# wei-zeng98/piano-a2s

Measured on AMD Instinct MI355X. Metric: training clips/sec (12 s, 5-bar), higher is better.
Workload: dtype f32

## Files before the change

piano_a2s_amd/csrc/a2s_api.hip:

```cpp
#define A2S_SWITCHES_IMPL
#include "a2s_internal.h"

thread_local char a2s_err_msg[512] = {0};
long long a2s_launch_counter = 0;

#define ST ((hipStream_t)stream)

extern "C" {

const char* a2s_last_error(void) { return a2s_err_msg; }
int a2s_version(void) { return 1; }
long long a2s_launch_count(void) { return __atomic_load_n(&a2s_launch_counter, __ATOMIC_RELAXED); }

int a2s_gemm_f32(void* stream, int M, int N, int K, float alpha, const float* A, long sAm, long sAk, const float* B, long sBk,
                 long sBn, float beta, float* C, long ldc, const float* bias, int act, int batch, long bsA, long bsB, long bsC,
                 int splitk, float* workspace, size_t workspace_bytes) {
    return a2s_gemm_impl(ST, M, N, K, alpha, A, sAm, sAk, B, sBk, sBn, beta, C, ldc, bias, act, batch, bsA, bsB, bsC, splitk,
                         workspace, workspace_bytes);
}
int a2s_gemm_f32_affine(void* stream, int M, int N, int K, float alpha, const float* A, long sAm, long sAk, const float* B, long sBk,
                        long sBn, float beta, float* C, long ldc, const float* bias, int act, int batch, long bsA, long bsB, long bsC,
                        int splitk, float* workspace, size_t workspace_bytes, const float* a_scale, const float* a_shift, int a_period,
                        const float* b_scale, const float* b_shift, int b_period) {
    return a2s_gemm_affine_impl(ST, M, N, K, alpha, A, sAm, sAk, B, sBk, sBn, beta, C, ldc, bias, act, batch, bsA, bsB, bsC, splitk,
// ... 30 lines not shown
                     const float* shift, int period, const float* dz_absmax, const float* y_absmax, float* workspace, size_t workspace_bytes) {
    return a2s_linear_wgrad_impl(ST, M, N, K, dz, ldz, y, lda, G, ldg, scale, shift, period, dz_absmax, y_absmax, workspace, workspace_bytes);
}
size_t a2s_linear_wgrad_ws_bytes(int M, int K) { return a2s_linear_wgrad_ws_bytes_impl(M, K); }
int a2s_linear_wgrad_eligible(int M, int N, int K, int period) { return a2s_linear_wgrad_ok(M, N, K, 256, 4, 4, period, nullptr, nullptr, nullptr) ? 1 : 0; }
int a2s_tallk_wgrad(void* stream, int M, int Np, int K, const float* P, long ldp, const float* A, long lda, float* G, long ldg, int transposed, float* bias,
                    const float* p_absmax, const float* a_absmax, float* workspace, size_t workspace_bytes) {
    return a2s_tallk_wgrad_impl(ST, M, Np, K, P, ldp, A, lda, G, ldg, transposed, bias, p_absmax, a_absmax, workspace, workspace_bytes);
}
size_t a2s_tallk_wgrad_ws_bytes(int M, int Np, int K) { return a2s_tallk_wgrad_ws_bytes_impl(M, Np, K); }
int a2s_tallk_wgrad_eligible(int M, int Np, int K, long ldp, long lda, long ldg, int transposed) {
    return a2s_tallk_wgrad_ok(M, Np, K, ldp, lda, ldg, transposed, nullptr, nullptr, nullptr, nullptr) ? 1 : 0;
}
int a2s_linear_fwd_eligible(int M, int N, int K, int period) { return a2s_linear_fwd_ok(M, N, K, 4, 4, period, nullptr, nullptr, nullptr) ? 1 : 0; }
int a2s_linear_dgrad_blocks(int M) { return a2s_linear_dgrad_blocks_impl(M); }
int a2s_linear_dgrad_eligible(int M, int N, int K, int period) {
    return a2s_linear_dgrad_ok(M, N, K, 4, 1, K, 4, period, nullptr, nullptr, nullptr, nullptr) ? 1 : 0;
}
int a2s_gemm_f32_bnstats(void* stream, int M, int N, int K, const float* A, long sAm, long sAk, const float* B, long sBk, long sBn, float* C, long ldc,
                         const float* y, const float* mean, const float* invstd, const float* scale, const float* shift, int period, float* partial) {
    return a2s_gemm_affine_impl(ST, M, N, K, 1.f, A, sAm, sAk, B, sBk, sBn, 0.f, C, ldc, nullptr, 0, 1, 0, 0, 0, 1, nullptr, 0,
                                nullptr, nullptr, 0, nullptr, nullptr, 0, y, mean, invstd, scale, shift, partial, period, 0, nullptr, nullptr);
}
int a2s_gemm_bnstats_blocks(int M, int period) { return a2s_cdiv(M, 128) * a2s_gemm_bnstats_slots(period); }
size_t a2s_gemm_workspace_bytes(int M, int N, int batch, int splitk) { return a2s_gemm_workspace_bytes_impl(M, N, batch, splitk); }
int a2s_gemm_pick_splitk(int M, int N, int K, int batch) { return a2s_gemm_pick_splitk_impl(M, N, K, batch); }
void a2s_gemm_debug_tile(int cfg) { a2s_gemm_debug_tile_impl(cfg); }
size_t a2s_note_step_workspace_floats(int H, int E) { return a2s_note_step_workspace_floats_impl(H, E); }
int a2s_debug_set(const char* key, int value) {
    if (!key) return A2S_ERR_ARG;
    const int id = a2s_switch_find(key);
    if (id >= 0) { a2s_switch_store(id, value); return A2S_OK; }
    if (!strcmp(key, "attn_deferred_fast")) { a2s_attn_deferred_fast = value ? 1 : 0; return A2S_OK; }
    if (!strcmp(key, "tallk_wgrad")) { a2s_tallk_wgrad_on = value ? 1 : 0; return A2S_OK; }
    if (!strcmp(key, "tallk_wgrad_max_splits")) { a2s_tallk_wgrad_max_splits = value > 0 ? value : 0; return A2S_OK; }
    if (!strcmp(key, "gemm_tile")) { a2s_gemm_debug_tile_impl(value); return A2S_OK; }
    snprintf(a2s_err_msg, sizeof(a2s_err_msg), "a2s_debug_set: unknown key %s", key);
    return A2S_ERR_ARG;
}
int a2s_env_check(void) {
    if (const char* e = a2s_switch_env_error()) A2S_FAIL(A2S_ERR_ARG, "%s: expected a decimal number >= 0", e);
    return A2S_OK;
}

int a2s_persist_abort_latch(void* device_word) { a2s_persist_latch_set(device_word); return A2S_OK; }

int a2s_debug_get(const char* key) {
    if (!key) return -1;
    const int id = a2s_switch_find(key);
    if (id == A2S_SW_attn_pair_fused_rows) return a2s_attn_pair_fused_rows();
    if (id >= 0) return a2s_sw((a2s_switch)id);
    if (!strcmp(key, "attn_pair_launches")) return (int)a2s_attn_pair_launches();
    if (!strcmp(key, "attn_pair_bwd_launches")) return (int)a2s_attn_pair_bwd_launches();
    if (!strcmp(key, "attn_deferred_fast")) return a2s_attn_deferred_fast;
    if (!strcmp(key, "tallk_wgrad")) return a2s_tallk_wgrad_on;
    if (!strcmp(key, "tallk_wgrad_max_splits")) return a2s_tallk_wgrad_max_splits;
    if (!strcmp(key, "tallk_wgrad_launches")) return (int)a2s_tallk_wgrad_launches();
    if (!strcmp(key, "attn_dk_ahead_launches")) return (int)a2s_attn_dk_ahead_launches();
    if (!strcmp(key, "attn_denc_launches")) return (int)a2s_attn_denc_launches();
    if (!strcmp(key, "dec_mid_launches")) return a2s_dec_mid_launches();
    if (!strcmp(key, "dec_cmb_launches")) return a2s_dec_cmb_launches();
    if (!strcmp(key, "dec_persist_launches")) return a2s_dec_persist_launches();
    if (!strcmp(key, "edit_distance_launches")) return (int)a2s_edit_distance_launches();
    if (!strcmp(key, "conv_rows16_c20_launches")) return (int)a2s_conv_rows16_c20_launches();
    if (!strcmp(key, "device_cus")) return a2s_device_geometry().cus;
    if (!strcmp(key, "device_xccs")) return a2s_device_geometry().xccs;
    return -1;
}

int a2s_conv3x3(void* stream, const float* x, const float* w, float* y, const float* in_scale, const float* in_shift,
                float* stat_partial, int B, int T, int F, int Cin, int Cout, int flip, float* workspace) {
    return a2s_conv3x3_impl(ST, x, w, y, in_scale, in_shift, stat_partial, B, T, F, Cin, Cout, flip, workspace, nullptr, nullptr, nullptr, nullptr, nullptr, nullptr,
                            nullptr, nullptr);
}
int a2s_conv3x3_ranged(void* stream, const float* x, const float* w, float* y, const float* in_scale, const float* in_shift, const float* in_absmax,
                       float* stat_partial, float* out_absmax, int B, int T, int F, int Cin, int Cout, float* workspace) {
    return a2s_conv3x3_impl(ST, x, w, y, in_scale, in_shift, stat_partial, B, T, F, Cin, Cout, 0, workspace, nullptr, nullptr, nullptr, nullptr, nullptr, nullptr,
                            in_absmax, out_absmax);
}
int a2s_conv3x3_dgrad_bnstats(void* stream, const float* dy, const float* w, float* g, const float* yl, const float* yl_mean, const float* yl_invstd,
                              const float* yl_scale, const float* yl_shift, float* stat_partial, int B, int T, int F, int Cin, int Cout,
                              float* workspace) {
    if (!yl) { snprintf(a2s_err_msg, sizeof(a2s_err_msg), "conv3x3_dgrad_bnstats: yl is required"); return A2S_ERR_ARG; }
    return a2s_conv3x3_impl(ST, dy, w, g, nullptr, nullptr, stat_partial, B, T, F, Cin, Cout, 1, workspace, yl, yl_mean, yl_invstd, yl_scale, yl_shift, nullptr, nullptr, nullptr);
}
int a2s_conv3x3_dgrad_bnstats_scaled(void* stream, const float* dy, const float* w, float* g, const float* yl, const float* yl_mean, const float* yl_invstd,
                                     const float* yl_scale, const float* yl_shift, float* stat_partial, int B, int T, int F, int Cin, int Cout,
                                     float* workspace, const float* dy_absmax) {
    if (!yl) { snprintf(a2s_err_msg, sizeof(a2s_err_msg), "conv3x3_dgrad_bnstats_scaled: yl is required"); return A2S_ERR_ARG; }
    return a2s_conv3x3_impl(ST, dy, w, g, nullptr, nullptr, stat_partial, B, T, F, Cin, Cout, 1, workspace, yl, yl_mean, yl_invstd, yl_scale, yl_shift, dy_absmax, nullptr, nullptr);
}
int a2s_conv3x3_dgrad_bnstats_ranged(void* stream, const float* dy, const float* w, float* g, const float* yl, const float* yl_mean, const float* yl_invstd,
                                     const float* yl_scale, const float* yl_shift, float* stat_partial, int B, int T, int F, int Cin, int Cout,
                                     float* workspace, const float* dy_absmax, float* g_absmax_out) {
    if (!yl) { snprintf(a2s_err_msg, sizeof(a2s_err_msg), "conv3x3_dgrad_bnstats_ranged: yl is required"); return A2S_ERR_ARG; }
    return a2s_conv3x3_impl(ST, dy, w, g, nullptr, nullptr, stat_partial, B, T, F, Cin, Cout, 1, workspace, yl, yl_mean, yl_invstd, yl_scale, yl_shift, dy_absmax, nullptr, g_absmax_out);
}
int a2s_bn_bwd_from_partial(void* stream, const float* g, const float* x, const float* mean, const float* invstd, const float* scale, const float* shift,
                            float* dgamma, float* dbeta, float* dx, const float* partial, int nblocks, float* c12, long rows, int C, int F) {
    return a2s_bn_bwd_from_partial_impl(ST, g, x, mean, invstd, scale, shift, dgamma, dbeta, dx, partial, nblocks, c12, rows, C, F, nullptr);
}
int a2s_bn_bwd_from_partial_amax(void* stream, const float* g, const float* x, const float* mean, const float* invstd, const float* scale, const float* shift,
                                 float* dgamma, float* dbeta, float* dx, const float* partial, int nblocks, float* c12, long rows, int C, int F,
                                 float* dx_absmax) {
    return a2s_bn_bwd_from_partial_impl(ST, g, x, mean, invstd, scale, shift, dgamma, dbeta, dx, partial, nblocks, c12, rows, C, F, dx_absmax);
}
// ... 360 lines not shown
```

piano_a2s_amd/csrc/a2s_bwd.hip:

```cpp
#include "a2s_internal.h"

__global__ __launch_bounds__(256) void log_softmax_bwd_rows(const float* __restrict__ g, const float* __restrict__ y,
                                                            long outer_stride, int inner, float* __restrict__ dx,
                                                            int R, int V, int n_outer, int time_major) {
    const int row = blockIdx.x * 4 + (threadIdx.x >> 6), lane = threadIdx.x & 63;
    if (row >= R) return;
    const int ob = row / inner, in = row % inner;
    const float* gr = g + (long)ob * outer_stride + (long)in * V;
    const float* yr = y + (long)ob * outer_stride + (long)in * V;
    float s = 0.f;
    for (int j = lane; j < V; j += 64) s += gr[j];
    s = wave_sum(s);
    const long orow = time_major ? ((long)in * n_outer + ob) : row;
    for (int j = lane; j < V; j += 64) dx[orow * V + j] = gr[j] - expf(yr[j]) * s;
}

int a2s_log_softmax_bwd_rows_impl(hipStream_t st, const float* g, const float* y, long outer_stride, int inner, float* dx,
                                  int R, int V, int n_outer, int time_major) {
    hipLaunchKernelGGL(log_softmax_bwd_rows, dim3(a2s_cdiv(R, 4)), dim3(256), 0, st, g, y, outer_stride, inner, dx, R, V, n_outer, time_major);
    A2S_CHECK_LAUNCH("log_softmax_bwd_rows");
    return A2S_OK;
}

__global__ void gru_gates_bwd(const float* __restrict__ dh_a, long lda, const float* __restrict__ dh_b, long ldb,
// ... 1086 lines not shown
    auto tile = [&](const f32x4 (&k)[4]) {
#pragma unroll
        for (int j = 0; j < NQ; ++j) {
            if (!on[j]) continue;
#pragma unroll
            for (int u = 0; u < 4; ++u) {
                const float w = dsv[j * chunk + i + 4 * u];
#pragma unroll
                for (int c = 0; c < 4; ++c) acc[j][c] = fmaf(w, sech2_ek(k[u][c], q4[j][c]), acc[j][c]);
            }
        }
    };
#pragma unroll
    for (int p = 0; p < KPRE; ++p)
        if (i + 12 < n) { tile(kpre[p]); i += 16; }
    for (; i + 12 < n; i += 16) {
        f32x4 k[4];
#pragma unroll
        for (int u = 0; u < 4; ++u) k[u] = ld_kv<NT>(Kb + (long)(i + 4 * u) * H + c4 * 4);
        tile(k);
    }
    for (; i < n; i += 4) {
        const f32x4 k0 = ld_kv<NT>(Kb + (long)i * H + c4 * 4);
#pragma unroll
        for (int j = 0; j < NQ; ++j) {
            if (!on[j]) continue;
            const float w = dsv[j * chunk + i];
#pragma unroll
            for (int c = 0; c < 4; ++c) acc[j][c] = fmaf(w, sech2_ek(k0[c], q4[j][c]), acc[j][c]);
        }
    }
    if (rg > 0) {
#pragma unroll
        for (int j = 0; j < NQ; ++j) red4[(j * 3 + rg - 1) * 64 + c4] = acc[j];
    }
    __syncthreads();
    if (rg == 0) {
        const f32x4 v4 = {v[c4 * 4], v[c4 * 4 + 1], v[c4 * 4 + 2], v[c4 * 4 + 3]};
#pragma unroll
        for (int j = 0; j < NQ; ++j) {
            if (!on[j]) continue;
            f32x4 a = acc[j];
#pragma unroll
            for (int u = 0; u < 3; ++u) { const f32x4 o = red4[(j * 3 + u) * 64 + c4];
#pragma unroll
                for (int c = 0; c < 4; ++c) a[c] += o[c]; }
#pragma unroll
            for (int c = 0; c < 4; ++c) a[c] *= v4[c];
            *reinterpret_cast<f32x4*>(dq_partial + (((long)slot * NQ + j) * G + g) * H + c4 * 4) = a;
        }
    }
}

struct AttnPairBwdSide { const float* Kmat; const float* q; const float* v; const float* attw; const float* ctx; const float* dctx_a; const float* dctx_b;
                         float* dctx_out; float* dq_partial; float* ds_out; const int* row_until; };
template <int NQ, bool NT>
__global__ __launch_bounds__(256, ATT_BWD_MQ_WAVES) void attn_bwd_split256_pair(AttnPairBwdSide s0, AttnPairBwdSide s1, const float* __restrict__ enc, long ldq,
                                                                                 long ldctx, long ldda, long lddb, long lddo, int T, int G, int chunk,
                                                                                 const int* __restrict__ clip_order, int step, int n_clips) {
    constexpr int H = 256, NJ = 2 * NQ;
    extern __shared__ __attribute__((aligned(16))) float sm[];
    float* dsv = sm;
    f32x4* red4 = reinterpret_cast<f32x4*>(sm + NJ * chunk);
    const int slot = blockIdx.x / G, g = blockIdx.x % G;
    const int b = clip_order ? clip_order[slot] : slot;
    const int t0 = g * chunk, t1 = min(T, t0 + chunk), n = t1 - t0;
    const int tid = threadIdx.x, lane = tid & 63, wave = tid >> 6;
    int onmask = 0;
#pragma unroll
    for (int j = 0; j < NQ; ++j) {
        onmask |= (!s0.row_until || step < s0.row_until[j * n_clips + b]) ? (1 << j) : 0;
        onmask |= (!s1.row_until || step < s1.row_until[j * n_clips + b]) ? (1 << (NQ + j)) : 0;
    }
    const float* Eb = enc + ((long)b * T + t0) * 2 * H;
    float* dcT = reinterpret_cast<float*>(red4);
    float* dots = dcT + NJ * ATT_DCS;
    for (int j = wave; j < NJ; j += 4) {
        const AttnPairBwdSide& sd = j < NQ ? s0 : s1;
        const int jr = j < NQ ? j : j - NQ;
        f32x4 d0 = {0.f, 0.f, 0.f, 0.f}, d1 = {0.f, 0.f, 0.f, 0.f};
        float dot = 0.f;
        if ((onmask >> j) & 1) {
            const long row = (long)jr * n_clips + b;
            d0 = *reinterpret_cast<const f32x4*>(sd.dctx_a + row * ldda + lane * 4);
            d1 = *reinterpret_cast<const f32x4*>(sd.dctx_a + row * ldda + H + lane * 4);
            if (sd.dctx_b) {
                const f32x4 o0 = *reinterpret_cast<const f32x4*>(sd.dctx_b + row * lddb + lane * 4);
                const f32x4 o1 = *reinterpret_cast<const f32x4*>(sd.dctx_b + row * lddb + H + lane * 4);
#pragma unroll
                for (int c = 0; c < 4; ++c) { d0[c] += o0[c]; d1[c] += o1[c]; }
            }
            if (sd.dctx_out && g == 0) {
                *reinterpret_cast<f32x4*>(sd.dctx_out + row * lddo + lane * 4) = d0;
                *reinterpret_cast<f32x4*>(sd.dctx_out + row * lddo + H + lane * 4) = d1;
            }
            const f32x4 c0 = *reinterpret_cast<const f32x4*>(sd.ctx + row * ldctx + lane * 4);
            const f32x4 c1 = *reinterpret_cast<const f32x4*>(sd.ctx + row * ldctx + H + lane * 4);
#pragma unroll
            for (int c = 0; c < 4; ++c) dot += d0[c] * c0[c] + d1[c] * c1[c];
            dot = wave_sum(dot);
        }
        *reinterpret_cast<f32x4*>(dcT + j * ATT_DCS + lane * 4) = d0;
        *reinterpret_cast<f32x4*>(dcT + j * ATT_DCS + H + lane * 4) = d1;
        if (lane == 0) dots[j] = dot;
    }
    __syncthreads();
// ... 116 lines not shown
        __syncthreads();
        if (rg == 0) {
            const f32x4 v4 = {sd.v[c4 * 4], sd.v[c4 * 4 + 1], sd.v[c4 * 4 + 2], sd.v[c4 * 4 + 3]};
#pragma unroll
            for (int j = 0; j < NQ; ++j) {
                if (!((smask >> j) & 1)) continue;
                f32x4 a = acc[j];
#pragma unroll
                for (int u = 0; u < 3; ++u) { const f32x4 o = red4[(j * 3 + u) * 64 + c4];
#pragma unroll
                    for (int c = 0; c < 4; ++c) a[c] += o[c]; }
#pragma unroll
                for (int c = 0; c < 4; ++c) a[c] *= v4[c];
                *reinterpret_cast<f32x4*>(sd.dq_partial + (((long)slot * NQ + j) * G + g) * H + c4 * 4) = a;
            }
        }
    }
}

__global__ __launch_bounds__(256) void attn_bwd_combine256(const float* __restrict__ dq_partial, float* __restrict__ dq, long lddq, int G,
                                                           const int* __restrict__ clip_rank, const int* __restrict__ row_until,
                                                           int n_clips, int groups, int n_active, int step, float* __restrict__ ds_out,
                                                           int T, float* __restrict__ dctx_out, long lddo) {
    const int b = blockIdx.x, j = threadIdx.x;
    const int clip = b % n_clips, grp = b / n_clips;
    const int slot = clip_rank ? clip_rank[clip] : clip;
    if (slot >= n_active || (row_until && step >= row_until[b])) {
        dq[(long)b * lddq + j] = 0.f;
        if (ds_out) for (int t = j; t < T; t += 256) ds_out[(long)b * T + t] = 0.f;
        if (dctx_out) for (int d = j; d < 512; d += 256) dctx_out[(long)b * lddo + d] = 0.f;
        return;
    }
    const float* pb = dq_partial + ((long)slot * groups + grp) * G * 256;
    float s = 0.f;
    for (int g0 = 0; g0 < G; g0 += 8) {
        float p[8];
#pragma unroll
        for (int u = 0; u < 8; ++u) p[u] = (g0 + u < G) ? pb[(long)(g0 + u) * 256 + j] : 0.f;
#pragma unroll
        for (int u = 0; u < 8; ++u) s += p[u];
    }
    dq[(long)b * lddq + j] = s;
}

template <int NQ>
static void launch_bwd_mq(hipStream_t st, int nwg, size_t shm, const float* Kmat, const float* enc, const float* q, long ldq, const float* v,
                          const float* attw, const float* ctx, long ldctx, const float* dctx_a, long ldda, const float* dctx_b, long lddb,
                          float* dctx_out, long lddo, float* ws, float* ds_out, int T, int G, int chunk, const a2s_attn_rows& r, bool nt) {
    if (nt) hipLaunchKernelGGL((attn_bwd_split256_mq<NQ, true>), dim3(nwg), dim3(256), shm, st, Kmat, enc, q, ldq, v, attw, ctx, ldctx, dctx_a, ldda, dctx_b, lddb,
                               dctx_out, lddo, ws, ds_out, T, G, chunk, r.clip_order, r.row_until, r.step, r.n_clips);
    else hipLaunchKernelGGL((attn_bwd_split256_mq<NQ, false>), dim3(nwg), dim3(256), shm, st, Kmat, enc, q, ldq, v, attw, ctx, ldctx, dctx_a, ldda, dctx_b, lddb,
                            dctx_out, lddo, ws, ds_out, T, G, chunk, r.clip_order, r.row_until, r.step, r.n_clips);
}

static int attn_step_bwd_split_impl(hipStream_t st, const float* Kmat, const float* enc, const float* q, long ldq, const float* v,
                                 const float* attw, const float* ctx, long ldctx, const float* dctx_a, long ldda, const float* dctx_b,
                                 long lddb, float* dctx_out, long lddo, float* dq, long lddq, float* ds_out, float* ws, int B, int T, int H,
                                 const a2s_attn_rows* rows) {
    A2S_REQUIRE(H == 256 && ws, "attn_step_bwd_split: needs hidden_size 256 and a workspace");
    A2S_REQUIRE(ldq % 4 == 0 && ldctx % 4 == 0 && ldda % 4 == 0 && (!dctx_b || lddb % 4 == 0) && (!dctx_out || lddo % 4 == 0),
                "attn_step_bwd_split: row strides must be multiples of 4 floats");
    A2S_REQUIRE(((uintptr_t)q | (uintptr_t)ctx | (uintptr_t)dctx_a | (uintptr_t)dctx_b | (uintptr_t)dctx_out | (uintptr_t)Kmat | (uintptr_t)enc) % 16 == 0,
                "attn_step_bwd_split: 16-byte alignment");
    a2s_attn_rows r = {nullptr, nullptr, nullptr, B, B, 0};
    if (rows) r = *rows;
    A2S_REQUIRE(r.n_clips > 0 && B % r.n_clips == 0, "attn_step_bwd_split: rows (%d) must be a multiple of the clips (%d)", B, r.n_clips);
    const int groups = B / r.n_clips;
    A2S_REQUIRE(groups <= A2S_ATTN_MAX_GROUPS, "attn_step_bwd_split: at most %d fused bars (got %d)", A2S_ATTN_MAX_GROUPS, groups);
    A2S_REQUIRE(r.n_active >= 0 && r.n_active <= r.n_clips && (!r.clip_order || r.clip_rank), "attn_step_bwd_split: bad row compaction");
    int G = 1, chunk = T;
    ws += A2S_ATTN_TICKETS;
    const bool nt = a2s_sw(A2S_SW_attn_nt) > 0 && r.n_active >= a2s_sw(A2S_SW_attn_nt) && groups == 1;
    if (r.n_active > 0) {
        a2s_attn_split_geometry(r.n_active, T, &G, &chunk);
        {
            const int fine = 4;
            if (fine > 0 && r.n_active <= fine && G == a2s_attn_max_split() && 2 * G <= 64) {
                int c = (T + 2 * G - 1) / (2 * G);
                c = (c + 3) & ~3;
                G = (T + c - 1) / c;
                chunk = c;
            }
        }
        const int nwg = r.n_active * G;
        if (groups == 1) {
            const size_t shm = a2s_attn_bulk_lds((chunk + 3 * 64 * 4) * sizeof(float), r.n_active, 1);
            if (nt) hipLaunchKernelGGL(attn_bwd_split256<true>, dim3(nwg), dim3(256), shm, st, Kmat, enc, q, ldq, v, attw, ctx, ldctx, dctx_a, ldda, dctx_b, lddb,
                                       dctx_out, lddo, ws, ds_out, T, G, chunk, r.clip_order);
            else hipLaunchKernelGGL(attn_bwd_split256<false>, dim3(nwg), dim3(256), shm, st, Kmat, enc, q, ldq, v, attw, ctx, ldctx, dctx_a, ldda, dctx_b, lddb,
                                    dctx_out, lddo, ws, ds_out, T, G, chunk, r.clip_order);
        } else {
            const size_t scratch = (size_t)groups * 3 * 64 * 4 > (size_t)groups * ATT_DCS + 16 ? (size_t)groups * 3 * 64 * 4 : (size_t)groups * ATT_DCS + 16;
            const size_t shm = a2s_attn_bulk_lds(((size_t)groups * chunk + scratch) * sizeof(float), r.n_active, 3);
#define A2S_BWD_MQ(N) launch_bwd_mq<N>(st, nwg, shm, Kmat, enc, q, ldq, v, attw, ctx, ldctx, dctx_a, ldda, dctx_b, lddb, dctx_out, lddo, ws, ds_out, T, G, chunk, r, nt)
            switch (groups) {
                case 2: A2S_BWD_MQ(2); break;
                case 3: A2S_BWD_MQ(3); break;
                case 4: A2S_BWD_MQ(4); break;
                default: A2S_BWD_MQ(5); break;
            }
#undef A2S_BWD_MQ
        }
        A2S_CHECK_LAUNCH("attn_bwd_split256");
    }
    hipLaunchKernelGGL(attn_bwd_combine256, dim3(B), dim3(256), 0, st, ws, dq, lddq, G, r.clip_rank, r.row_until, r.n_clips, groups, r.n_active, r.step,
                       ds_out, T, dctx_out, lddo);
    A2S_CHECK_LAUNCH("attn_bwd_combine256");
    return A2S_OK;
}

template <int NQ>
static void launch_bwd_pair(hipStream_t st, int nwg, size_t shm, const AttnPairBwdSide& s0, const AttnPairBwdSide& s1, const float* enc, long ldq, long ldctx,
                            long ldda, long lddb, long lddo, int T, const AttnPairStep& p) {
    hipLaunchKernelGGL((attn_bwd_split256_pair<NQ, false>), dim3(nwg), dim3(256), shm, st, s0, s1, enc, ldq, ldctx, ldda, lddb, lddo, T, p.G, p.chunk,
                       p.clip_order, p.step, p.n_clips);
}
static long g_attn_pair_bwd_launches = 0;
long a2s_attn_pair_bwd_launches(void) { return g_attn_pair_bwd_launches; }

static AttnPairBwdSide attn_pair_bwd_side(const a2s_note_dec_bwd_args& a, int s) {
    const int H2 = 2 * a.H, ldx = a.E + H2;
    const long R = a.R;
    return AttnPairBwdSide{a.keys, a.q + (long)s * R * a.H, a.attn_v, a.attw + (long)s * R * a.T, a.x + (long)s * R * ldx + a.E, a.dx + (long)s * R * ldx + a.E,
                           a.do_all + (long)s * R * 2 * H2 + H2, a.dctx_all + (long)s * R * H2, a.attn_ws + A2S_ATTN_TICKETS, a.ds_all + (long)s * R * a.T, a.row_until};
}

static int attn_pair_bwd_sweep(hipStream_t st, const a2s_note_dec_bwd_args& au, const a2s_note_dec_bwd_args& al, int s, AttnPairStep& p) {
    const int T = au.T, H2 = 2 * au.H, ldx = au.E + H2, groups = au.R / p.n_clips;
    A2S_REQUIRE(au.H == 256 && au.E == al.E && au.enc == al.enc && au.R == al.R && groups >= 1 && groups <= A2S_ATTN_MAX_GROUPS && ldx % 4 == 0,
                "attn_pair_bwd_sweep: the staves must decode the same rows over the same encoder outputs");
    a2s_attn_split_geometry(p.n_active, T, &p.G, &p.chunk);
    const AttnPairBwdSide s0 = attn_pair_bwd_side(au, s), s1 = attn_pair_bwd_side(al, s);
    const size_t red = (size_t)groups * 3 * 64 * 4, img = (size_t)2 * groups * ATT_DCS + 16;
    const size_t shm = a2s_attn_bulk_lds(((size_t)2 * groups * p.chunk + (red > img ? red : img)) * sizeof(float), p.n_active, 3);
    const int nwg = p.n_active * p.G;
#define A2S_BWD_PAIR(N) launch_bwd_pair<N>(st, nwg, shm, s0, s1, au.enc, au.H, ldx, ldx, 2 * H2, H2, T, p)
    switch (groups) {
        case 1: A2S_BWD_PAIR(1); break;
// ... 20 lines not shown
```

piano_a2s_amd/csrc/a2s_internal.h:

```cpp
#pragma once
#include "a2s_common.h"
#include "../../include/a2s.h"
#include "a2s_switches.h"

static inline int a2s_attn_pair_fused_rows(void) {
    const int cap = a2s_sw(A2S_SW_dec_fused_max_rows), v = a2s_sw(A2S_SW_attn_pair_fused_rows);
    return v < cap ? v : cap;
}
static inline unsigned a2s_persist_dbg(void) {
    return (a2s_sw(A2S_SW_persist_force_agent) ? PERSIST_DBG_FORCE_AGENT : 0u) | (a2s_sw(A2S_SW_persist_inject_abort) ? PERSIST_DBG_INJECT_ABORT : 0u);
}

int a2s_absmax_impl(hipStream_t st, const float* x, long n, float* out);
size_t a2s_gemm_workspace_bytes_impl(int M, int N, int batch, int splitk);
int a2s_gemm_pick_splitk_impl(int M, int N, int K, int batch);
int a2s_gemm_bnstats_slots(int period);
void a2s_gemm_debug_tile_impl(int cfg);
int a2s_gemm_affine_impl(hipStream_t st, int M, int N, int K, float alpha, const float* A, long sAm, long sAk,
    const float* B, long sBk, long sBn, float beta, float* C, long ldc, const float* bias, int act,
    int batch, long bsA, long bsB, long bsC, int splitk, float* ws, size_t ws_bytes,
    const float* a_scale, const float* a_shift, int a_period, const float* b_scale, const float* b_shift, int b_period,
    const float* ep_y, const float* ep_mean, const float* ep_invstd, const float* ep_scale, const float* ep_shift,
    float* ep_partial, int ep_period, int two_term, const float* a_absmax, const float* b_absmax);
int a2s_gemm_impl(hipStream_t st, int M, int N, int K, float alpha, const float* A, long sAm, long sAk,
// ... 106 lines not shown
int a2s_embed_rows_impl(hipStream_t st, const float* table, const long long* ids64, const int* ids32, long id_stride,
    int const_id, float* out, long ldo, int col0, int R, int E, const uint8_t* drop, float inv_keep);
int a2s_note_decoder_fwd_impl(hipStream_t st, const a2s_note_dec_args& a, int* steps_done);
int a2s_note_decoder_fwd_grammar_impl(hipStream_t st, const a2s_note_dec_args& a, const a2s_grammar_ref& g, int* steps_done);
int a2s_note_decoder_fwd_metre_impl(hipStream_t st, const a2s_note_dec_args& a, const a2s_grammar_ref& g, const a2s_metre_ref* mt, int* steps_done);
int a2s_note_decoder_fwd_pair_impl(hipStream_t su, hipStream_t sl, const a2s_note_dec_args& au, const a2s_note_dec_args& al, const int* pair_order,
    const int* pair_rank, const int* pair_n_active, int* done_u, int* done_l);
int a2s_staff_emb_fwd_impl(hipStream_t st, const float* note_emb, const float* const* w ,
    const long long* ids64, const int* ids32, long id_bstride, const long long* lengths,
    long len_stride, float* out, long ldo, int col0, float* hsave, int R, int maxlen, int E, int S);
int a2s_note_decoder_zero_unwritten(hipStream_t st, const a2s_note_dec_args& a, const char* who );
size_t a2s_attn_workspace_floats_impl(int B, int T, int H, int groups);
size_t a2s_attn_bulk_lds(size_t shm, int n_active, int backward);
long a2s_attn_pair_launches(void);
struct AttnPairStep { const int* clip_order; const int* clip_rank; int n_clips; int n_active; int step; int G; int chunk; };
int a2s_pair_events(const char* who, hipEvent_t** ev_out);
static inline int a2s_record_wait(hipEvent_t ev, hipStream_t from, hipStream_t to, const char* who) {
    hipError_t e = hipEventRecord(ev, from);
    if (e == hipSuccess) e = hipStreamWaitEvent(to, ev, 0);
    if (e != hipSuccess) A2S_FAIL(A2S_ERR_HIP, "%s: event: %s", who, hipGetErrorString(e));
    return A2S_OK;
}

int a2s_log_softmax_bwd_rows_impl(hipStream_t st, const float* g, const float* y, long outer_stride, int inner, float* dx,
    int R, int V, int n_outer, int time_major);
int a2s_gru_gates_bwd_impl(hipStream_t st, const float* dh_a, long lda, const float* dh_b, long ldb, const float* save,
    const float* hprev, long ldhp, float* dgi, long ldgi, float* dgh, long ldgh, float* dgh2, long ldgh2,
    float* dhprev, long lddp, int R, int H);
int a2s_attn_step_bwd_impl(hipStream_t st, const float* Kmat, const float* enc, const float* q, long ldq, const float* v,
    const float* attw, const float* ctx, long ldctx, const float* dctx_a, long ldda, const float* dctx_b,
    long lddb, float* dctx_out, long lddo, float* dq, long lddq, float* ds_out, int B, int T, int H, float* ws,
    const a2s_attn_rows* rows = nullptr);
int a2s_attn_dk_accum_impl(hipStream_t st, const float* Kmat, const float* q_all, const float* ds_all, const float* v,
    float* dK, float* dv_partial, int B, int T, int S, int H, const int* row_until, int groups);
int a2s_attn_denc_accum_impl(hipStream_t st, const float* attw_all, const float* dctx_all, float* dEnc, int B, int T, int S, int H2,
    const int* row_until, int groups);
long a2s_attn_dk_ahead_launches(void);
long a2s_attn_denc_launches(void);
int a2s_col_sum_impl(hipStream_t st, const float* x, long ld, float* out, long rows, int C, float alpha, float beta, float* ws, size_t ws_floats);
int a2s_embed_scatter_add_impl(hipStream_t st, float* table_grad, const long long* ids64, const int* ids32, long id_stride,
    int const_id, const float* g, long ldg, int col0, int R, int E, const uint8_t* drop, float inv_keep);
int a2s_ew_act_bwd_impl(hipStream_t st, const float* g, const float* y, float* dx, long n, int act);
int a2s_note_decoder_bwd_impl(hipStream_t st, const a2s_note_dec_bwd_args& a);
int a2s_note_decoder_bwd_pair_impl(hipStream_t su, hipStream_t sl, const a2s_note_dec_bwd_args& au, const a2s_note_dec_bwd_args& al, const int* pair_order,
    const int* pair_rank, const int* pair_n_active);
int a2s_gru_seq_bwd_impl(hipStream_t st, const float* dout, long do_bstride, long do_tstride, const float* out, long out_bstride,
    long out_tstride, const float* gates, const float* w_hh, const float* dhn, float* dgi_all, float* dgh_shift,
    float* dgh_first, float* dhbuf, float* dgh_tmp, int B, int T, int H, int reverse, float* ws, size_t ws_bytes,
    float* ranges_out, int* ranges_valid);
int a2s_staff_emb_bwd_impl(hipStream_t st, const float* note_emb, const float* const* w, float* const* grads_dev, float* note_emb_grad,
    const long long* ids64, const int* ids32, long id_bstride, const long long* lengths, long len_stride,
    const float* dout, long lddo, int col0, const float* hsave, int R, int maxlen, int E, int S);
long a2s_attn_pair_bwd_launches(void);

size_t a2s_note_step_fused_head_floats(void);
size_t a2s_note_step_workspace_floats_impl(int H, int E);
int a2s_dec_mid_launches(void);
int a2s_dec_cmb_launches(void);
bool a2s_dec_step_fusable(int R, int H, int E, int V, const void* const* ptrs, int nptrs, const float* ws, size_t ws_floats, bool greedy = false);
int a2s_note_step_fused_fwd(hipStream_t st, const a2s_note_dec_args& a, int si, int so, int sv, int sv_next, int t, const int* t_base, int tf, bool last,
    int nrows, const int* rowmap, const a2s_attn_deferred* defer = nullptr);
int a2s_note_step_fused_bwd_prepare(hipStream_t st, const a2s_note_dec_bwd_args& a);
int a2s_note_step_fused_bwd(hipStream_t st, const a2s_note_dec_bwd_args& a, int s, const float* dh_in, float* dh_out, const a2s_attn_rows* rows,
    int nrows, const int* rowmap);
bool a2s_note_step_mid_ok(int H, int E, const void* const* ptrs, int nptrs);
int a2s_note_step_mid_gru(hipStream_t st, const a2s_note_dec_args& a, int si, int so, int sv, int sv_next, int nrows, const int* rowmap);
bool a2s_note_step_mid_bwd_ok(const a2s_note_dec_bwd_args& a);
int a2s_note_step_mid_bwd(hipStream_t st, const a2s_note_dec_bwd_args& a, int s, float* dh_out, int nrows, const int* rowmap);
int a2s_note_step_mid_bwd_query(hipStream_t st, const a2s_note_dec_bwd_args& a, int s, float* dh_out, int nrows, const int* rowmap);

bool a2s_grammar_ref_ok(const a2s_grammar_ref& g, int R, int V);
int a2s_grammar_argmax_rows_impl(hipStream_t st, const float* x, long ldx, float* y, long ldy, const signed char* next, int n_states, int* row_state,
    int* choice_out, int R, int V);
int a2s_grammar_step_finalize_impl(hipStream_t st, const StepFinArgs& a, const a2s_grammar_ref& g);
int a2s_grammar_launches_impl(void);
bool a2s_metre_ref_ok(const a2s_metre_ref& m);
int a2s_metre_argmax_rows_impl(hipStream_t st, const float* x, long ldx, float* y, long ldy, const signed char* next, int n_states, int* row_state,
    const a2s_metre_ref* mt, int* choice_out, int R, int V);
int a2s_metre_step_finalize_impl(hipStream_t st, const StepFinArgs& a, const a2s_grammar_ref& g, const a2s_metre_ref& mt);
int a2s_metre_launches_impl(void);

int a2s_attn_align_rows_impl(hipStream_t st, const float* attw, long ldw, int R, int T, int* peak_out, float* weight_out, float* centroid_out,
    long out_stride, const int* n_done = nullptr, int n_rows_total = 0);
int a2s_align_launches_impl(void);
int a2s_note_decoder_fwd_align_impl(hipStream_t st, const a2s_note_dec_args& a, const a2s_align_args& g, int* steps_done);

int a2s_render_notes_impl(hipStream_t st, const int* programs, int rows_per_clip, int n_samples, float* wave, long wave_bstride, int B);
int a2s_render_launches_impl(void);

int a2s_transpose_targets_impl(hipStream_t st, const int* new_key, const int* interval, const int* token_map, int n_rows, int V, const int* semitones,
    const float* detune, long long* key, long long* upper, long long* lower, int bars, int U, int L, int bins_per_semitone, float* eff_bins, int* counters,
    int B);
int a2s_shift_bins_impl(hipStream_t st, const float* x, float* y, const float* eff_bins, int B, int rows, int F);
int a2s_augment_launches_impl(void);

#define A2S_ROW_TX 128
#define A2S_ROW_TY 2
#define A2S_ROW_TILE 16
#define A2S_ROW_NR (A2S_ROW_TILE / A2S_ROW_TY)
#ifdef __HIPCC__
template <int VEC> struct a2s_row_vec { typedef float type; };
template <> struct a2s_row_vec<4> { typedef f32x4 type; };
static inline int a2s_row_vec_width(int F, const void* y) { return (F % 4 == 0 && ((uintptr_t)y & 15) == 0) ? 4 : 1; }
static inline bool a2s_row_grid(int B, int rows, int F, int vec, dim3* grid) {
    *grid = dim3(a2s_cdiv(rows, A2S_ROW_TILE), B, a2s_cdiv(F, A2S_ROW_TX * vec));
    return grid->z <= 65535;
// ... 140 lines not shown
```

piano_a2s_amd/csrc/a2s_switches.h:

```cpp
#pragma once
#include <stdio.h>
#include <stdlib.h>
#include <string.h>

#define A2S_SWITCHES(X)                                                                                                                              \
     \
    X(conv_rows, 7, COUNT, "A2S_CONV_ROWS")                                                                                                          \
                                                                         \
    X(wgrad_rows, 1, COUNT, "A2S_WGRAD_ROWS")                                                                                                        \
             \
    X(conv_c1_fast, 1, RAW, 0)                                                                                                                       \
           \
    X(conv_bf16x3, 3, RAW, 0)                                                                                                                        \
                              \
    X(conv_f16x2, 3, COUNT, 0)                                                                                                                       \
                                  \
    X(wgrad_bf16x3, 1, RAW, 0)                                                                                                                       \
                                                                \
    X(wgrad_f16x2, 1, COUNT, 0)                                                                                                                      \
                                      \
    X(gemm_bf16x3, 1, RAW, 0)                                                                                                                        \
                                      \
    X(gemm_f16x2, 1, COUNT, 0)                                                                                                                       \
                                                                  \
    X(gru_fused, 1, ONOFF, 0)                                                                                                                        \
                                                    \
    X(gru_persist, 1, ONOFF, "A2S_GRU_PERSIST")                                                                                                      \
                              \
    X(gru_persist_alone, 0, ONOFF, 0)                                                                                                                \
                                                                              \
    X(staff_emb_fast, 1, ONOFF, 0)                                                                                                                   \
                                                                                       \
    X(dec_fused, 1, ONOFF, "A2S_DEC_FUSED")                                                                                                          \
                                                                                           \
    X(dec_fused_max_rows, 192, COUNT, 0)                                                                                                             \
                  \
    X(attn_pair_fused_rows, 32, RAW, 0)                                                                                                              \
                                             \
    X(dec_mid, 1, ONOFF, 0)                                                                                                                          \
                                          \
    X(dec_persist, 1, ONOFF, "A2S_DEC_PERSIST")                                                                                                      \
                                               \
    X(attn_pair, 1, ONOFF, 0)                                                                                                                        \
                                          \
    X(attn_deep, 24, COUNT, 0)                                                                                                                       \
                                                              \
    X(attn_defer_combine, 1, ONOFF, 0)                                                                                                               \
      \
    X(attn_fused_combine, 0, COUNT, 0)                                                                                                               \
                                          \
    X(attn_nt, 64, COUNT, 0)                                                                                                                         \
             \
    X(attn_bulk_cap, 0, ONOFF, 0)                                                                                                                    \
                                  \
    X(persist_force_agent, 0, ONOFF, 0)                                                                                                              \
                                                                                 \
    X(persist_inject_abort, 0, ONOFF, 0)

enum a2s_switch {
#define X(key, def, rule, env) A2S_SW_##key,
    A2S_SWITCHES(X)
#undef X
    A2S_SW_COUNT
};
extern int a2s_switch_value[A2S_SW_COUNT];
static inline int a2s_sw(a2s_switch id) { return a2s_switch_value[id]; }

extern int a2s_attn_deferred_fast;

int a2s_switch_find(const char* key);
void a2s_switch_store(int id, int value);
const char* a2s_switch_env_error(void);

#ifdef A2S_SWITCHES_IMPL
enum { A2S_RULE_ONOFF, A2S_RULE_COUNT, A2S_RULE_RAW };
struct a2s_switch_desc { const char* key; int rule; const char* env; };
static const a2s_switch_desc a2s_switch_table[A2S_SW_COUNT] = {
#define X(key, def, rule, env) {#key, A2S_RULE_##rule, env},
    A2S_SWITCHES(X)
#undef X
};
int a2s_switch_value[A2S_SW_COUNT] = {
#define X(key, def, rule, env) def,
    A2S_SWITCHES(X)
#undef X
};
static char a2s_switch_bad_env[96] = {0};

int a2s_switch_find(const char* key) {
    for (int i = 0; key && i < A2S_SW_COUNT; ++i)
        if (!strcmp(key, a2s_switch_table[i].key)) return i;
    return -1;
}
void a2s_switch_store(int id, int value) {
    const int rule = a2s_switch_table[id].rule;
    a2s_switch_value[id] = rule == A2S_RULE_ONOFF ? (value ? 1 : 0) : (rule == A2S_RULE_COUNT && value < 0) ? 0 : value;
}
// ... 18 lines not shown
```

Before: 635.7.

## Add deep register-resident attention backward kernel for small active batches

Adds an attention-step backward kernel for small numbers of active clips. It preloads encoder and key rows into registers, computes the score gradients for multi-query groups with 16x16x4 f32 MFMA, and uses finer time chunks so more workgroups fill the CUs. It is selected when the active count is at or below the attn_deep threshold, the chunk is small and the workgroup count fits within the CU count. The cost is heavy register use, which may lower occupancy, plus more partial sums for the dq combine.

```diff
diff --git a/piano_a2s_amd/csrc/a2s_api.hip b/piano_a2s_amd/csrc/a2s_api.hip
--- a/piano_a2s_amd/csrc/a2s_api.hip
+++ b/piano_a2s_amd/csrc/a2s_api.hip
@@ -106,6 +106,7 @@
     if (id >= 0) return a2s_sw((a2s_switch)id);
     if (!strcmp(key, "attn_pair_launches")) return (int)a2s_attn_pair_launches();
     if (!strcmp(key, "attn_pair_bwd_launches")) return (int)a2s_attn_pair_bwd_launches();
+    if (!strcmp(key, "attn_deep_bwd_launches")) return (int)a2s_attn_deep_bwd_launches();
     if (!strcmp(key, "attn_deferred_fast")) return a2s_attn_deferred_fast;
     if (!strcmp(key, "tallk_wgrad")) return a2s_tallk_wgrad_on;
     if (!strcmp(key, "tallk_wgrad_max_splits")) return a2s_tallk_wgrad_max_splits;
diff --git a/piano_a2s_amd/csrc/a2s_bwd.hip b/piano_a2s_amd/csrc/a2s_bwd.hip
--- a/piano_a2s_amd/csrc/a2s_bwd.hip
+++ b/piano_a2s_amd/csrc/a2s_bwd.hip
@@ -1162,6 +1162,201 @@
     }
 }
 
+template <int NQ>
+__global__ __launch_bounds__(256) void attn_bwd_split256_deep(const float* __restrict__ Kmat, const float* __restrict__ enc,
+                                                              const float* __restrict__ q, long ldq, const float* __restrict__ v,
+                                                              const float* __restrict__ attw, const float* __restrict__ ctx, long ldctx,
+                                                              const float* __restrict__ dctx_a, long ldda, const float* __restrict__ dctx_b, long lddb,
+                                                              float* __restrict__ dctx_out, long lddo, float* __restrict__ dq_partial,
+                                                              float* __restrict__ ds_out, int T, int G, int chunk,
+                                                              const int* __restrict__ clip_order, const int* __restrict__ row_until,
+                                                              int step, int n_clips) {
+    constexpr int H = 256, KF = 10;
+    extern __shared__ __attribute__((aligned(16))) float sm[];
+    float* dsv = sm;
+    f32x4* red4 = reinterpret_cast<f32x4*>(sm + NQ * chunk);
+    float* dcT = reinterpret_cast<float*>(red4);
+    float* dots = dcT + NQ * ATT_DCS;
+    const int slot = blockIdx.x / G, g = blockIdx.x % G;
+    const int b = clip_order ? clip_order[slot] : slot;
+    const int t0 = g * chunk, t1 = min(T, t0 + chunk), n = t1 - t0;
+    const int tid = threadIdx.x, lane = tid & 63, wave = tid >> 6;
+    const int li = lane & 15, lg = lane >> 4, lr = min(li, NQ - 1);
+    const int c4 = lane, rg = wave;
+    const float* Kb = Kmat + ((long)b * T + t0) * H;
+    const float* Eb = enc + ((long)b * T + t0) * 2 * H;
+    int until = 0x7fffffff;
+    if (row_until) until = row_until[min(lane, NQ - 1) * n_clips + b];
+    const long roww = (long)min(wave, NQ - 1) * n_clips + b;
+    f32x4 d0 = *reinterpret_cast<const f32x4*>(dctx_a + roww * ldda + lane * 4);
+    f32x4 d1 = *reinterpret_cast<const f32x4*>(dctx_a + roww * ldda + H + lane * 4);
+    f32x4 o0 = {0.f, 0.f, 0.f, 0.f}, o1 = {0.f, 0.f, 0.f, 0.f};
+    if (dctx_b) {
+        o0 = *reinterpret_cast<const f32x4*>(dctx_b + roww * lddb + lane * 4);
+        o1 = *reinterpret_cast<const f32x4*>(dctx_b + roww * lddb + H + lane * 4);
+    }
+    const f32x4 c0 = *reinterpret_cast<const f32x4*>(ctx + roww * ldctx + lane * 4);
+    const f32x4 c1 = *reinterpret_cast<const f32x4*>(ctx + roww * ldctx + H + lane * 4);
+    const long arow = ((long)lr * n_clips + b) * T + t0;
+    constexpr int AF = 12;
+    float aw[NQ == 1 ? AF : 4];
+    const bool ablk = wave * 16 < n;
+    const int fr = wave * 16 + li;
+    const bool valid = fr < n;
+    f32x4 e[32];
+    if constexpr (NQ == 1) {
+#pragma unroll
+        for (int m = 0; m < AF; ++m) aw[m] = attw[arow + min(wave * 4 + (m & 3) + 16 * (m >> 2), n - 1)];
+#pragma unroll
+        for (int m = 0; m < AF; ++m) {
+            const float* ep = Eb + (long)min(wave * 4 + (m & 3) + 16 * (m >> 2), n - 1) * 2 * H + lane * 4;
+            e[2 * m] = *reinterpret_cast<const f32x4*>(ep);
+            e[2 * m + 1] = *reinterpret_cast<const f32x4*>(ep + H);
+        }
+    } else {
+#pragma unroll
+        for (int r = 0; r < 4; ++r) aw[r] = attw[arow + min(wave * 16 + 4 * lg + r, n - 1)];
+        if (ablk) {
+            const float* ep = Eb + (long)min(fr, n - 1) * 2 * H + 8 * lg;
+#pragma unroll
+            for (int u = 0; u < 16; ++u) {
+                e[2 * u] = *reinterpret_cast<const f32x4*>(ep + 32 * u);
+                e[2 * u + 1] = *reinterpret_cast<const f32x4*>(ep + 32 * u + 4);
+            }
+        }
+    }
+    f32x4 k[KF];
+#pragma unroll
+    for (int u = 0; u < KF; ++u) k[u] = *reinterpret_cast<const f32x4*>(Kb + (long)min(rg + 4 * u, n - 1) * H + c4 * 4);
+    f32x4 q4[NQ];
+#pragma unroll
+    for (int j = 0; j < NQ; ++j) q4[j] = *reinterpret_cast<const f32x4*>(q + ((long)j * n_clips + b) * ldq + c4 * 4);
+    const f32x4 v4 = {v[c4 * 4], v[c4 * 4 + 1], v[c4 * 4 + 2], v[c4 * 4 + 3]};
+    const int onmask = (int)(__builtin_amdgcn_ballot_w64(step < until) & ((1u << NQ) - 1));
+    if constexpr (NQ == 1) {
+        if (onmask) {
+            if (dctx_b) {
+#pragma unroll
+                for (int c = 0; c < 4; ++c) { d0[c] += o0[c]; d1[c] += o1[c]; }
+            }
+            if (dctx_out && g == 0 && wave == 0) {
+                *reinterpret_cast<f32x4*>(dctx_out + roww * lddo + lane * 4) = d0;
+                *reinterpret_cast<f32x4*>(dctx_out + roww * lddo + H + lane * 4) = d1;
+            }
+            float dot_ctx = 0.f;
+#pragma unroll
+            for (int c = 0; c < 4; ++c) dot_ctx += d0[c] * c0[c] + d1[c] * c1[c];
+            dot_ctx = wave_sum(dot_ctx);
+#pragma unroll
+            for (int m = 0; m < AF; ++m) {
+                const int f2 = wave * 4 + (m & 3) + 16 * (m >> 2);
+                float s = 0.f;
+#pragma unroll
+                for (int c = 0; c < 4; ++c) s += d0[c] * e[2 * m][c] + d1[c] * e[2 * m + 1][c];
+                s = wave_sum_lane63(s);
+                if (lane == 63 && f2 < n) {
+                    const float d_s = aw[m] * (s - dot_ctx);
+                    dsv[f2] = d_s;
+                    if (ds_out) ds_out[arow + f2] = d_s;
+                }
+            }
+        }
+    } else {
+    if (wave < NQ) {
+        float dot = 0.f;
+        if ((onmask >> wave) & 1) {
+            if (dctx_b) {
+#pragma unroll
+                for (int c = 0; c < 4; ++c) { d0[c] += o0[c]; d1[c] += o1[c]; }
+            }
+            if (dctx_out && g == 0) {
+                *reinterpret_cast<f32x4*>(dctx_out + roww * lddo + lane * 4) = d0;
+                *reinterpret_cast<f32x4*>(dctx_out + roww * lddo + H + lane * 4) = d1;
+            }
+#pragma unroll
+            for (int c = 0; c < 4; ++c) dot += d0[c] * c0[c] + d1[c] * c1[c];
+            dot = wave_sum(dot);
+        } else {
+            d0 = d1 = (f32x4){0.f, 0.f, 0.f, 0.f};
+        }
+        *reinterpret_cast<f32x4*>(dcT + wave * ATT_DCS + lane * 4) = d0;
+        *reinterpret_cast<f32x4*>(dcT + wave * ATT_DCS + H + lane * 4) = d1;
+        if (lane == 0) dots[wave] = dot;
+    }
+    __syncthreads();
+    if (ablk) {
+        const float* brow = dcT + lr * ATT_DCS + 8 * lg;
+        const float dotn = dots[lr];
+        const bool mine = li < NQ && ((onmask >> li) & 1);
+        f32x4 acc = {0.f, 0.f, 0.f, 0.f}, acc2 = {0.f, 0.f, 0.f, 0.f};
+#pragma unroll
+        for (int u = 0; u < 16; ++u) {
+            f32x4 e0 = e[2 * u], e1 = e[2 * u + 1];
+            if (!valid) e0 = e1 = (f32x4){0.f, 0.f, 0.f, 0.f};
+            const f32x4 b0 = *reinterpret_cast<const f32x4*>(brow + 32 * u);
+            const f32x4 b1 = *reinterpret_cast<const f32x4*>(brow + 32 * u + 4);
+#pragma unroll
+            for (int c = 0; c < 4; ++c) acc = __builtin_amdgcn_mfma_f32_16x16x4f32(e0[c], b0[c], acc, 0, 0, 0);
+#pragma unroll
+            for (int c = 0; c < 4; ++c) acc2 = __builtin_amdgcn_mfma_f32_16x16x4f32(e1[c], b1[c], acc2, 0, 0, 0);
+        }
+#pragma unroll
+        for (int r = 0; r < 4; ++r) acc[r] += acc2[r];
+        if (mine) {
+#pragma unroll
+            for (int r = 0; r < 4; ++r) {
+                const int f2 = wave * 16 + 4 * lg + r;
+                if (f2 < n) {
+                    const float d_s = aw[r] * (acc[r] - dotn);
+                    dsv[li * chunk + f2] = d_s;
+                    if (ds_out) ds_out[arow + f2] = d_s;
+                }
+            }
+        }
+    }
+    }
+    __syncthreads();
+    f32x4 acc[NQ];
+#pragma unroll
+    for (int j = 0; j < NQ; ++j) {
+        acc[j] = (f32x4){0.f, 0.f, 0.f, 0.f};
+#pragma unroll
+        for (int c = 0; c < 4; ++c) q4[j][c] = exp2x_clamped(q4[j][c]);
+    }
+#pragma unroll
+    for (int u = 0; u < KF; ++u) {
+        const int i = rg + 4 * u;
+        if (i < n) {
+#pragma unroll
+            for (int j = 0; j < NQ; ++j) {
+                if (!((onmask >> j) & 1)) continue;
+                const float w = dsv[j * chunk + i];
+#pragma unroll
+                for (int c = 0; c < 4; ++c) acc[j][c] = fmaf(w, sech2_ek(k[u][c], q4[j][c]), acc[j][c]);
+            }
+        }
+    }
+    if (rg > 0) {
+#pragma unroll
+        for (int j = 0; j < NQ; ++j) red4[(j * 3 + rg - 1) * 64 + c4] = acc[j];
+    }
+    __syncthreads();
+    if (rg == 0) {
+#pragma unroll
+        for (int j = 0; j < NQ; ++j) {
+            if (!((onmask >> j) & 1)) continue;
+            f32x4 a = acc[j];
+#pragma unroll
+            for (int u = 0; u < 3; ++u) { const f32x4 o = red4[(j * 3 + u) * 64 + c4];
+#pragma unroll
+                for (int c = 0; c < 4; ++c) a[c] += o[c]; }
+#pragma unroll
+            for (int c = 0; c < 4; ++c) a[c] *= v4[c];
+            *reinterpret_cast<f32x4*>(dq_partial + (((long)slot * NQ + j) * G + g) * H + c4 * 4) = a;
+        }
+    }
+}
+
 struct AttnPairBwdSide { const float* Kmat; const float* q; const float* v; const float* attw; const float* ctx; const float* dctx_a; const float* dctx_b;
                          float* dctx_out; float* dq_partial; float* ds_out; const int* row_until; };
 template <int NQ, bool NT>
@@ -1384,6 +1579,18 @@
     else hipLaunchKernelGGL((attn_bwd_split256_mq<NQ, false>), dim3(nwg), dim3(256), shm, st, Kmat, enc, q, ldq, v, attw, ctx, ldctx, dctx_a, ldda, dctx_b, lddb,
                             dctx_out, lddo, ws, ds_out, T, G, chunk, r.clip_order, r.row_until, r.step, r.n_clips);
 }
+
+template <int NQ>
+static void launch_bwd_deep(hipStream_t st, int nwg, const float* Kmat, const float* enc, const float* q, long ldq, const float* v,
+                            const float* attw, const float* ctx, long ldctx, const float* dctx_a, long ldda, const float* dctx_b, long lddb,
+                            float* dctx_out, long lddo, float* ws, float* ds_out, int T, int G, int chunk, const a2s_attn_rows& r) {
+    const size_t scratch = (size_t)NQ * 3 * 64 * 4 > (size_t)NQ * ATT_DCS + 16 ? (size_t)NQ * 3 * 64 * 4 : (size_t)NQ * ATT_DCS + 16;
+    const size_t shm = ((size_t)NQ * chunk + scratch) * sizeof(float);
+    hipLaunchKernelGGL((attn_bwd_split256_deep<NQ>), dim3(nwg), dim3(256), shm, st, Kmat, enc, q, ldq, v, attw, ctx, ldctx, dctx_a, ldda, dctx_b, lddb,
+                       dctx_out, lddo, ws, ds_out, T, G, chunk, r.clip_order, r.row_until, r.step, r.n_clips);
+}
+static long g_attn_deep_bwd_launches = 0;
+long a2s_attn_deep_bwd_launches(void) { return g_attn_deep_bwd_launches; }
 
 static int attn_step_bwd_split_impl(hipStream_t st, const float* Kmat, const float* enc, const float* q, long ldq, const float* v,
                                  const float* attw, const float* ctx, long ldctx, const float* dctx_a, long ldda, const float* dctx_b,
@@ -1405,17 +1612,31 @@
     const bool nt = a2s_sw(A2S_SW_attn_nt) > 0 && r.n_active >= a2s_sw(A2S_SW_attn_nt) && groups == 1;
     if (r.n_active > 0) {
         a2s_attn_split_geometry(r.n_active, T, &G, &chunk);
+        bool deep = groups <= 4 && r.n_active <= a2s_sw(A2S_SW_attn_deep) && chunk <= 80;
         {
             const int fine = 4;
-            if (fine > 0 && r.n_active <= fine && G == a2s_attn_max_split() && 2 * G <= 64) {
-                int c = (T + 2 * G - 1) / (2 * G);
-                c = (c + 3) & ~3;
-                G = (T + c - 1) / c;
-                chunk = c;
-            }
+            const bool finer = fine > 0 && r.n_active <= fine && G == a2s_attn_max_split() && 2 * G <= 64;
+            int Gf = G, cf = chunk;
+            if ((finer || (deep && chunk > 40)) && 2 * G <= 64) {
+                cf = (T + 2 * G - 1) / (2 * G);
+                cf = (cf + 3) & ~3;
+                Gf = (T + cf - 1) / cf;
+            }
+            deep = deep && cf <= 40 && r.n_active * Gf <= a2s_device_geometry().cus;
+            if (finer || deep) { G = Gf; chunk = cf; }
         }
         const int nwg = r.n_active * G;
-        if (groups == 1) {
+        if (deep) {
+#define A2S_BWD_DEEP(N) launch_bwd_deep<N>(st, nwg, Kmat, enc, q, ldq, v, attw, ctx, ldctx, dctx_a, ldda, dctx_b, lddb, dctx_out, lddo, ws, ds_out, T, G, chunk, r)
+            switch (groups) {
+                case 1: A2S_BWD_DEEP(1); break;
+                case 2: A2S_BWD_DEEP(2); break;
+                case 3: A2S_BWD_DEEP(3); break;
+                default: A2S_BWD_DEEP(4); break;
+            }
+#undef A2S_BWD_DEEP
+            __atomic_fetch_add(&g_attn_deep_bwd_launches, 1, __ATOMIC_RELAXED);
+        } else if (groups == 1) {
             const size_t shm = a2s_attn_bulk_lds((chunk + 3 * 64 * 4) * sizeof(float), r.n_active, 1);
             if (nt) hipLaunchKernelGGL(attn_bwd_split256<true>, dim3(nwg), dim3(256), shm, st, Kmat, enc, q, ldq, v, attw, ctx, ldctx, dctx_a, ldda, dctx_b, lddb,
                                        dctx_out, lddo, ws, ds_out, T, G, chunk, r.clip_order);
diff --git a/piano_a2s_amd/csrc/a2s_internal.h b/piano_a2s_amd/csrc/a2s_internal.h
--- a/piano_a2s_amd/csrc/a2s_internal.h
+++ b/piano_a2s_amd/csrc/a2s_internal.h
@@ -182,6 +182,7 @@
     const long long* ids64, const int* ids32, long id_bstride, const long long* lengths, long len_stride,
     const float* dout, long lddo, int col0, const float* hsave, int R, int maxlen, int E, int S);
 long a2s_attn_pair_bwd_launches(void);
+long a2s_attn_deep_bwd_launches(void);
 
 size_t a2s_note_step_fused_head_floats(void);
 size_t a2s_note_step_workspace_floats_impl(int H, int E);
diff --git a/piano_a2s_amd/csrc/a2s_switches.h b/piano_a2s_amd/csrc/a2s_switches.h
--- a/piano_a2s_amd/csrc/a2s_switches.h
+++ b/piano_a2s_amd/csrc/a2s_switches.h
@@ -42,7 +42,7 @@
     X(dec_persist, 1, ONOFF, "A2S_DEC_PERSIST")                                                                                                      \
                                                \
     X(attn_pair, 1, ONOFF, 0)                                                                                                                        \
-                                          \
+                            \
     X(attn_deep, 24, COUNT, 0)                                                                                                                       \
                                                               \
     X(attn_defer_combine, 1, ONOFF, 0)                                                                                                               \
```

After: 638.0 (median of 6 runs). About the same (+0.4%).
